# eblerjana/pangenie

Hardware: AMD Instinct MI355X
Metric: genotyped variants/sec (whole node) at H haplotypes; HBM GB/s vs roofline (higher is better)
Workload: dtype f64

## Files before the change

### pangenie_amd/csrc/pg_experiments.h

```cpp
#pragma once

#ifndef PG_EXP
#define PG_EXP 0
#endif
static constexpr unsigned kExp = PG_EXP;
#ifdef PG_CHAIN_PROF
static constexpr bool kChainProf = true;
#else
static constexpr bool kChainProf = false;
#endif

#ifndef PG_LEAN_EXP
#define PG_LEAN_EXP 0
#endif
static constexpr unsigned kLeanExp = PG_LEAN_EXP;
#ifndef PG_LEAN_UPKEEP_EXP
#define PG_LEAN_UPKEEP_EXP 0
#endif
static constexpr unsigned kLeanUpkeepExp = PG_LEAN_UPKEEP_EXP;
#ifdef PG_LEAN_DPPSUM
static constexpr bool kLeanDppSum = true;
#else
static constexpr bool kLeanDppSum = false;
#endif

#ifdef PG_POST_GENERIC
static constexpr bool kPostGeneric = true;
#else
static constexpr bool kPostGeneric = false;
#endif

#ifndef PG_PERSIST_EXP
#define PG_PERSIST_EXP 0
#endif
static constexpr unsigned kPersistExp = PG_PERSIST_EXP;

#ifndef PG_LEAN_PRETOTAL
#define PG_LEAN_PRETOTAL 0
#endif
static constexpr bool kLeanPreTotal = PG_LEAN_PRETOTAL != 0;

#ifdef PG_NT_STORES
static constexpr bool kNtStores = true;
#else
static constexpr bool kNtStores = false;
#endif
#ifdef PG_NT_POST
static constexpr bool kNtPost = true;
#else
static constexpr bool kNtPost = false;
#endif

#ifndef PG_LX_EXP
#define PG_LX_EXP 0
#endif
static constexpr unsigned kLxExp = PG_LX_EXP;

#ifndef PG_LEANP_EXP
#define PG_LEANP_EXP 0
#endif
static constexpr unsigned kLeanpExp = PG_LEANP_EXP;

#ifdef PG_LEAN_TIMELINE
static constexpr bool kLeanTimeline = true;
#else
static constexpr bool kLeanTimeline = false;
#endif
struct LeanTimeline {
    unsigned long long t[10], acc[10];
    DEVI void init() { if constexpr (kLeanTimeline) { for (int i = 0; i < 10; ++i) { t[i] = 0; acc[i] = 0; } } }
    template <int I>
    DEVI void mark(double dep) {
        if constexpr (kLeanTimeline) {
            __builtin_amdgcn_sched_barrier(0);
            asm volatile("" :: "v"(dep));
            t[I] = __builtin_amdgcn_s_memtime();
            __builtin_amdgcn_sched_barrier(0);
        }
    }
    template <int N>
    DEVI void fold() {
        if constexpr (kLeanTimeline) {
#pragma unroll
            for (int i = 0; i < N; ++i) acc[i] += t[i + 1] - t[i];
            acc[9] += 1;
        }
    }
    DEVI void write(unsigned long long* o) const {
        if constexpr (kLeanTimeline) { for (int i = 0; i < 9; ++i) o[i] = acc[i]; o[15] = acc[9]; }
    }
};

#ifndef PG_X_EXP
#define PG_X_EXP 0
#endif
static constexpr unsigned kXExp = PG_X_EXP;

#ifdef PG_VIT_TIMELINE
static constexpr bool kVitTimeline = true;
#else
static constexpr bool kVitTimeline = false;
#endif
// ... 38 lines not shown
```

### pangenie_amd/csrc/pg_kernels.hip

```cpp
#include <hip/hip_runtime.h>
#include <math.h>
#include <stdint.h>
#include <stdlib.h>

#include <type_traits>

#include "pg_device.h"
#include "pg_devmath.h"
#include "pg_launch.h"

#define DEVI __device__ __forceinline__
typedef double v2f64 __attribute__((ext_vector_type(2)));
#include "pg_experiments.h"

template <int CTRL, int ROW_MASK, bool BOUND>
DEVI double dpp_f64(double v) {
    int lo = __double2loint(v), hi = __double2hiint(v);
    lo = __builtin_amdgcn_update_dpp(0, lo, CTRL, ROW_MASK, 0xF, BOUND);
    hi = __builtin_amdgcn_update_dpp(0, hi, CTRL, ROW_MASK, 0xF, BOUND);
    return __hiloint2double(hi, lo);
}

DEVI double readlane_f64(double v, int src_lane ) {
    int lo = __builtin_amdgcn_readlane(__double2loint(v), src_lane);
// ... 2431 lines not shown
    static constexpr int NW = 64 / R;
    double psum[2][NW][64];
    double ptot[2][NW] __attribute__((aligned(32)));
    double u[NW][64] __attribute__((aligned(16)));
    double scal[2][64];
    double img[2 * PG_LEAN_BLOCK][PG_LEAN_IMAGE / 8] __attribute__((aligned(PG_LEAN_IMAGE)));
};
static_assert(PG_LEAN_IMAGE == 256 && (2 * PG_LEAN_BLOCK * PG_LEAN_IMAGE & (2 * PG_LEAN_BLOCK * PG_LEAN_IMAGE - 1)) == 0, "image(rel): a shift and a mask");
constexpr uint32_t kLeanImgTab = 64u, kLeanImgComb = 192u;
template <class SH>
DEVI LAS const unsigned char* lean_image(const SH& sh, uint32_t rel ) {
    static_assert(sizeof(sh.img) == 2u * PG_LEAN_SPARSE * PG_LEAN_IMAGE, "pg_lean_ring_image");
    return (LAS const unsigned char*)&sh.img[0][0] + pg_lean_ring_image(rel);
}
struct FRec {
    double c0, c1, c2, kappa, E00, E01, E11;
    unsigned long long bits1;
};
typedef double v4f64 __attribute__((ext_vector_type(4)));
struct LeanRecs {
    const GAS char* base;
    int64_t origin, C;
    int dir;
    uint32_t tid;
    DEVI v2f64 fetch(uint32_t block) const {
        int64_t c = origin + (int64_t)dir * ((int64_t)block * PG_LEAN_BLOCK + ((tid & 255u) >> 2));
        c = c < 0 ? 0 : (c >= C ? C - 1 : c);
        return *(const GAS v2f64*)(base + (size_t)c * 64u + (tid & 3u) * 16u);
    }
    template <class SH>
    DEVI void park(SH& sh, uint32_t block, v2f64 piece) const {
        if (tid < 256u) *(v2f64*)&sh.img[(block & 1u) * PG_LEAN_BLOCK + (tid >> 2)][(tid & 3u) * 2u] = piece;
    }
};
template <class SH>
DEVI FRec read_frec(const SH& sh, uint32_t rel ) {
    LAS const double* q = (LAS const double*)lean_image(sh, rel);
    FRec r;
    r.c0 = q[0]; r.c1 = q[1]; r.c2 = q[2]; r.kappa = q[3]; r.E00 = q[4]; r.E01 = q[5]; r.E11 = q[6];
    r.bits1 = (unsigned long long)__double_as_longlong(q[7]);
    return r;
}

DEVI double wave_total_mfma(double v) {
    const v4f64 z = {0.0, 0.0, 0.0, 0.0};
    const v4f64 a = __builtin_amdgcn_mfma_f64_16x16x4f64(v, 1.0, z, 0, 0, 0);
    const double u = (a[0] + a[1]) + (a[2] + a[3]);
    const v4f64 b = __builtin_amdgcn_mfma_f64_16x16x4f64(u, 1.0, z, 0, 0, 0);
    return b[0];
}
DEVI double sel_by_bit(uint32_t bits , int k, double if0, double if1) {
    const uint32_t m = (uint32_t)(((int32_t)(bits << (31 - k))) >> 31);
    const uint32_t lo = ((uint32_t)__double2loint(if1) & m) | ((uint32_t)__double2loint(if0) & ~m);
    const uint32_t hi = ((uint32_t)__double2hiint(if1) & m) | ((uint32_t)__double2hiint(if0) & ~m);
    return __hiloint2double((int)hi, (int)lo);
}

struct ColScalars {
    double* row;
    unsigned long long valid = 0ull;
    DEVI void put(uint32_t , uint64_t t , double v ) {
        row[t & 63u] = v;
        valid |= 1ull << (t & 63u);
    }
    DEVI void flush(gdouble* arr, uint32_t lane, uint64_t t_any ) {
        if ((valid >> lane) & 1ull) arr[(t_any & ~(uint64_t)63u) + lane] = row[lane];
        valid = 0ull;
    }
};

template <int R>
DEVI void lean_u_rows(double urep, double (&ui)[R]) {
    static_assert(R == 16, "one DPP row of 16 lanes = the wave's 16 rows");
    ui[0] = row_bcast_f64<0>(urep);   ui[1] = row_bcast_f64<1>(urep);   ui[2] = row_bcast_f64<2>(urep);   ui[3] = row_bcast_f64<3>(urep);
    ui[4] = row_bcast_f64<4>(urep);   ui[5] = row_bcast_f64<5>(urep);   ui[6] = row_bcast_f64<6>(urep);   ui[7] = row_bcast_f64<7>(urep);
    ui[8] = row_bcast_f64<8>(urep);   ui[9] = row_bcast_f64<9>(urep);   ui[10] = row_bcast_f64<10>(urep); ui[11] = row_bcast_f64<11>(urep);
    ui[12] = row_bcast_f64<12>(urep); ui[13] = row_bcast_f64<13>(urep); ui[14] = row_bcast_f64<14>(urep); ui[15] = row_bcast_f64<15>(urep);
}
template <int K>
DEVI double fmac_row_bcast(double acc, double u, double s) {
    asm("v_fmac_f64_dpp %0, %1, %2 row_newbcast:%3 row_mask:0xf bank_mask:0xf" : "+v"(acc) : "v"(u), "v"(s), "n"(K));
    return acc;
}
DEVI void pin_here(double& v) { asm volatile("" : "+v"(v)); }
DEVI void lean_fence() { __builtin_amdgcn_sched_barrier(0); }
DEVI double dpp_source(double v) {
    double r;
    asm("v_mov_b64 %0, %1\n\ts_nop 1" : "=v"(r) : "v"(v));
    return r;
}
template <int K>
DEVI unsigned long long row_mask64(unsigned long long bits ) {
    unsigned long long m;
    asm("s_bfe_i64 %0, %1, %2" : "=s"(m) : "s"(bits), "n"((1 << 16) | K) : "scc");
    return m;
}
DEVI double sel_by_mask(double if0, double if1, unsigned long long m ) {
    uint32_t lo, hi;
    asm("v_cndmask_b32_e64 %0, %1, %2, %3" : "=v"(lo) : "v"(__double2loint(if0)), "v"(__double2loint(if1)), "s"(m));
    asm("v_cndmask_b32_e64 %0, %1, %2, %3" : "=v"(hi) : "v"(__double2hiint(if0)), "v"(__double2hiint(if1)), "s"(m));
    return __hiloint2double((int)hi, (int)lo);
}
template <int K, int N, class F>
DEVI void static_for(F&& f) {
    if constexpr (K < N) { f(std::integral_constant<int, K>{}); static_for<K + 1, N>(f); }
}
template <int SEL>
DEVI uint32_t add_byte(uint32_t bytes, uint32_t base) {
    uint32_t r;
    if constexpr (SEL == 0) asm("v_add_u32_sdwa %0, %1, %2 dst_sel:DWORD dst_unused:UNUSED_PAD src0_sel:BYTE_0 src1_sel:DWORD" : "=v"(r) : "v"(bytes), "v"(base));
    else if constexpr (SEL == 1) asm("v_add_u32_sdwa %0, %1, %2 dst_sel:DWORD dst_unused:UNUSED_PAD src0_sel:BYTE_1 src1_sel:DWORD" : "=v"(r) : "v"(bytes), "v"(base));
    else if constexpr (SEL == 2) asm("v_add_u32_sdwa %0, %1, %2 dst_sel:DWORD dst_unused:UNUSED_PAD src0_sel:BYTE_2 src1_sel:DWORD" : "=v"(r) : "v"(bytes), "v"(base));
    else asm("v_add_u32_sdwa %0, %1, %2 dst_sel:DWORD dst_unused:UNUSED_PAD src0_sel:BYTE_3 src1_sel:DWORD" : "=v"(r) : "v"(bytes), "v"(base));
    return r;
}
template <class SH>
DEVI void lean_expand(SH& sh, uint32_t block , uint32_t tid) {
    static_assert(sizeof(sh.img[0]) == PG_LEAN_IMAGE && kLeanImgComb + 4u * 8u <= PG_LEAN_IMAGE, "four waves of eight row pairs");
    if (tid >= 256u) return;
    double* im = sh.img[(block & 1u) * PG_LEAN_BLOCK + (tid >> 2)];
    {
        const uint32_t c = tid & 3u;
        const double E00 = im[4], E01 = im[5], E11 = im[6];
        v2f64* tab = (v2f64*)((unsigned char*)im + kLeanImgTab);
        tab[c * 2u + 0u] = v2f64{(c & 1u) ? E01 : E00, (c & 2u) ? E01 : E00};
        tab[c * 2u + 1u] = v2f64{(c & 1u) ? E11 : E01, (c & 2u) ? E11 : E01};
    }
    {
        const uint32_t w = tid & 3u;
        const unsigned long long bits = (unsigned long long)__double_as_longlong(im[7]);
        const uint32_t b16 = (uint32_t)(bits >> (16u * w)) & 0xFFFFu;
        auto spread = [](uint32_t v8) { return ((v8 & 3u) | (((v8 >> 2) & 3u) << 8) | (((v8 >> 4) & 3u) << 16) | (((v8 >> 6) & 3u) << 24)) << 5; };
        typedef uint32_t u32x2 __attribute__((ext_vector_type(2)));
        *(u32x2*)((unsigned char*)im + kLeanImgComb + w * 8u) = u32x2{spread(b16 & 0xFFu), spread(b16 >> 8)};
    }
}
struct LeanPairs { uint32_t tbase, cd0, cd1; };
typedef uint32_t u32x2 __attribute__((ext_vector_type(2)));
template <class SH>
DEVI u32x2 lean_pair_bytes(const SH& sh, uint32_t rel , uint32_t wave ) {
    return *(LAS const u32x2*)(lean_image(sh, rel) + kLeanImgComb + wave * 8u);
}
template <class SH>
DEVI LeanPairs lean_pairs(const SH& sh, uint32_t rel , u32x2 cd, uint32_t aj ) {
    return LeanPairs{(uint32_t)(uintptr_t)lean_image(sh, rel) + kLeanImgTab + aj * 16u, cd.x, cd.y};
}
template <class SH>
DEVI LeanPairs lean_pairs(const SH& sh, uint32_t rel, uint32_t wave, uint32_t aj) { return lean_pairs(sh, rel, lean_pair_bytes(sh, rel, wave), aj); }
template <int P>
DEVI v2f64 lean_pair(const LeanPairs& lp) {
    return *(LAS const v2f64*)(uintptr_t)add_byte<(P & 3)>(P < 4 ? lp.cd0 : lp.cd1, lp.tbase);
}
template <int R>
DEVI void lean_pairs_all(const LeanPairs& lp, double (&e)[R]) {
    static_for<0, R / 2>([&](auto pc) __attribute__((always_inline)) { constexpr int q = decltype(pc)::value; const v2f64 t = lean_pair<q>(lp); e[2 * q] = t.x; e[2 * q + 1] = t.y; });
}
template <class SH>
DEVI v2f64 lean_ring_open(SH& sh, const LeanRecs& recs, uint32_t s0 , uint32_t tid) {
    const bool two = s0 > PG_LEAN_RING_PARK;
    recs.park(sh, 0, recs.fetch(0));
    v2f64 piece = recs.fetch(1);
    if (two) {
        lds_barrier();
        lean_expand(sh, 0, tid);
        lds_barrier();
        recs.park(sh, 1, piece);
// ... 13 lines not shown
            recs.park(sh, blk, piece);
            piece = recs.fetch(blk + 1u);
        } else if (((n + 3u) % PG_LEAN_BLOCK) == 0u) {
            lean_expand(sh, (n + 3u) / PG_LEAN_BLOCK, tid);
        }
    } else if constexpr (UPKEEP == kUpkeepPark) {
        const uint32_t blk = (n + 4u) / PG_LEAN_BLOCK;
        recs.park(sh, blk, piece);
        piece = recs.fetch(blk + 1u);
    } else if constexpr (UPKEEP == kUpkeepExpand) {
        lean_expand(sh, (n + 3u) / PG_LEAN_BLOCK, tid);
    }
}
template <int R>
DEVI double lean_colsum(const LeanShared<R>& sh, uint32_t pb, uint32_t lane) {
    if constexpr (R == 16)
        return (sh.psum[pb][0][lane] + sh.psum[pb][1][lane]) + (sh.psum[pb][2][lane] + sh.psum[pb][3][lane]);
    else
        return ((sh.psum[pb][0][lane] + sh.psum[pb][1][lane]) + (sh.psum[pb][2][lane] + sh.psum[pb][3][lane])) +
               ((sh.psum[pb][4][lane] + sh.psum[pb][5][lane]) + (sh.psum[pb][6][lane] + sh.psum[pb][7][lane]));
}



#define PG_SYNC_TIMEOUT_TICKS 1000000000ull
#ifndef PG_POLL_SLEEPS
#define PG_POLL_SLEEPS 2
#endif
DEVI bool chunk_spin(uint32_t* flag, uint32_t want, uint32_t* err) {
    bool ok = __hip_atomic_load(flag, __ATOMIC_RELAXED, __HIP_MEMORY_SCOPE_AGENT) >= want;
    if (!ok) {
        const unsigned long long t0 = wall_clock64();
        for (uint32_t it = 0;; ++it) {
#pragma unroll
            for (int z = 0; z < PG_POLL_SLEEPS; ++z) __builtin_amdgcn_s_sleep(127);
            if (__hip_atomic_load(flag, __ATOMIC_RELAXED, __HIP_MEMORY_SCOPE_AGENT) >= want) { ok = true; break; }
            if ((it & 63u) == 63u) {
                if (__hip_atomic_load(err, __ATOMIC_RELAXED, __HIP_MEMORY_SCOPE_AGENT) & PG_DEVERR_SYNC_TIMEOUT) break;
                if (wall_clock64() - t0 > PG_SYNC_TIMEOUT_TICKS) { atomicOr(err, PG_DEVERR_SYNC_TIMEOUT); break; }
            }
        }
    }
    if (ok) __builtin_amdgcn_fence(__ATOMIC_ACQUIRE, "agent");
    return ok;
}
DEVI void chunk_publish(uint32_t* flag, uint32_t value) {
    __builtin_amdgcn_fence(__ATOMIC_RELEASE, "agent");
    __syncthreads();
    if (threadIdx.x == 0) __hip_atomic_store(flag, value, __ATOMIC_RELEASE, __HIP_MEMORY_SCOPE_AGENT);
}
DEVI void chunk_wait_buffer(uint32_t* flag, uint32_t want, uint32_t* err) {
    if (threadIdx.x == 0 && !(kPersistExp & 2u)) (void)chunk_spin(flag, want, err);
    __syncthreads();
}

DEVI void lean_store(gdouble2* p, v2f64 v) {
    if constexpr (kNtStores) __builtin_nontemporal_store(v, p);
    else *p = v;
}
template <int R>
DEVI void lean_put_sums(LeanShared<R>& sh, uint32_t pb, uint32_t wave, uint32_t lane, double part) {
    sh.psum[pb][wave][lane] = part;
    if constexpr (kLeanPreTotal) {
        double v = part;
        v += dpp_f64<0x111, 0xF, true>(v);
        v += dpp_f64<0x112, 0xF, true>(v);
        v += dpp_f64<0x114, 0xF, true>(v);
        v += dpp_f64<0x118, 0xF, true>(v);
        v += dpp_f64<0x142, 0xA, false>(v);
        v += dpp_f64<0x143, 0xC, false>(v);
        if (lane == 63u) sh.ptot[pb][wave] = v;
    }
}
template <int R>
DEVI double lean_total(const LeanShared<R>& sh, uint32_t pb) {
    static_assert(R == 16, "four waves");
    const v2f64 a = *(const v2f64*)&sh.ptot[pb][0], b = *(const v2f64*)&sh.ptot[pb][2];
    return (a.x + a.y) + (b.x + b.y);
}

template <int PHASE, int R, bool TRI, bool SPARSE = false>
DEVI void lean_forward(const DevContig& dc, LeanShared<R>& sh, uint32_t C, uint32_t chunk) {
    static_assert(!SPARSE || ((PHASE == 1 || PHASE == 3) && !TRI), "sparse stores: phases 1 and 3 of full-column lean chains");
    constexpr int HP = 64;
    constexpr uint32_t RMASK = (1u << R) - 1u;
    const uint32_t mid = C / 2, K = dc.chunk_cols;
    uint32_t lo = PHASE == 1 ? 0u : mid, hi = PHASE == 1 ? mid : C;
    if constexpr (PHASE == 3) {
        const unsigned long long l = (unsigned long long)mid + (unsigned long long)chunk * K;
        if (l >= C) return;
        lo = (uint32_t)l;
        hi = C - lo > K ? lo + K : C;
    }
    if constexpr (SPARSE && PHASE == 1) if (chunk) {
        uint32_t pc[2];
        if (!pg_sparse_piece(C, 0u, (chunk >> 16) * K, chunk & 0xFFFFu, pc)) return;
        lo = pc[0]; hi = pc[1] + 1u;
    }
    bool seg2 = false;
    if constexpr (PHASE == 5) {
        lo = chunk + 1u; hi = chunk + PG_LEAN_SPARSE;
        seg2 = lo >= mid;
        if (seg2) hi = C - lo > PG_LEAN_SPARSE ? lo + PG_LEAN_SPARSE : C;
    }
    if (lo >= hi) return;
    const uint32_t first = lo == 0 ? 1u : lo;
    const uint32_t tid = threadIdx.x, lane = tid & 63u;
    const uint32_t wave = __builtin_amdgcn_readfirstlane(tid >> 6);
    const uint32_t i0 = wave * R;
    const size_t colsz = TRI ? (size_t)dc.col_stride : (size_t)HP * HP;
    const double unif = 1.0 / 4096.0;
    const uint32_t s0 = SPARSE ? pg_lean_ring_first(pg_lean_ring_lead(C, 0u, (uint32_t)PHASE, first, hi)) : 0u;
    LeanRecs recs{(const GAS char*)dc.frec, (int64_t)first - 1 - (int64_t)s0, (int64_t)C, +1, tid};
    v2f64 piece = lean_ring_open(sh, recs, s0, tid);
    gdouble* fwd = (gdouble*)dc.fwd;
    gdouble* fscale = (gdouble*)dc.fscale;
    gu8* fallback = (gu8*)dc.fwd_fallback;
    gdouble* wr = fwd;
    gcdouble* resume = (gcdouble*)(fwd + (size_t)(lo > 0 ? lo - 1 : 0) * colsz);
    if constexpr (PHASE == 3) {
        gdouble* scr = (gdouble*)dc.scratch;
        wr = scr + (size_t)(PG_SCR_BUF(chunk) * 2u) * K * colsz - (size_t)lo * colsz;
        if constexpr (SPARSE) { if (chunk > 0) resume = (gcdouble*)dc.ckpt + (size_t)(lo - mid) / PG_LEAN_SPARSE * colsz; }
        else if (chunk > 0) resume = (gcdouble*)(scr + ((size_t)(PG_SCR_BUF(chunk - 1u) * 2u) * K + (K - 1u)) * colsz);
    }
    if constexpr (PHASE == 4) wr = (gdouble*)dc.scratch - (size_t)lo * colsz;
    bool boundary = false;
    if constexpr (PHASE == 5) if (seg2) {
        const uint32_t m = (lo - mid) / PG_LEAN_SPARSE, ci = (lo - mid) / K;
        if (m) resume = (gcdouble*)dc.ckpt + (size_t)m * colsz;
        wr = (gdouble*)dc.scratch + (size_t)(PG_SCR_BUF(ci) * 2u) * K * colsz - ((size_t)mid + (size_t)ci * K) * colsz;
        boundary = (lo - mid) % K == 0u;
    }
    const size_t toff = (size_t)(i0 >> 1) * HP + lane;
    auto emis = [&](const FRec& r, double& eA, double& eB) {
        const bool aj = (r.bits1 >> lane) & 1ull;
        eA = aj ? r.E01 : r.E00;
        eB = aj ? r.E11 : r.E01;
    };
    double tfa[TRI ? R / 2 : 1], tfb[TRI ? R / 2 : 1];
    uint32_t tskip = 0, tunit[TRI ? R / 2 : 1];
    uint32_t rskip = 0;
    if constexpr (PHASE == 5) {
#pragma unroll
        for (int q = 0; q < R / 2; ++q) rskip |= (lane < ((i0 + 2u * (uint32_t)q) & ~7u) ? 1u : 0u) << q;
    }
    if constexpr (TRI) {
#pragma unroll
        for (int q = 0; q < R / 2; ++q) {
            const uint32_t r0 = i0 + 2u * (uint32_t)q;
            tfa[q] = lane < r0 ? 0.0 : (lane == r0 ? 0.5 : 1.0);
            tfb[q] = lane <= r0 ? 0.0 : (lane == r0 + 1u ? 0.5 : 1.0);
            const bool off_q = lane < (r0 & ~7u);
            tskip |= (off_q ? 1u : 0u) << q;
            tunit[q] = off_q ? 0u : tri_unit_of(r0 >> 1, lane);
        }
    }
    auto put_pair = [&](gdouble2* dst, int q, double a, double b) __attribute__((always_inline)) {
        if constexpr (TRI) {
            if (!((tskip >> q) & 1u)) lean_store((dst - toff) + tunit[q], v2f64{a * tfa[q], b * tfb[q]});
        } else if constexpr (PHASE == 5) {
            if (!((rskip >> q) & 1u)) lean_store(dst + (size_t)q * HP, v2f64{a, b});
        } else {
            lean_store(dst + (size_t)q * HP, v2f64{a, b});
        }
    };
    auto col_at = [&](uint32_t c) __attribute__((always_inline)) -> gdouble* {
        if constexpr (SPARSE && PHASE == 3) return (gdouble*)dc.ckpt + (size_t)((c - (mid - 1u)) / PG_LEAN_SPARSE) * colsz;
        else return wr + (size_t)c * colsz;
    };
    auto store_col = [&](uint32_t c, const double (&v)[R]) {
        gdouble2* dst = (gdouble2*)col_at(c) + toff;
#pragma unroll
        for (int k = 0; k < R; k += 2) put_pair(dst, k >> 1, v[k], v[k + 1]);
    };
    auto flag_uniform = [&](uint32_t cprev) {
        bool stored = cprev >= lo;
        if constexpr (SPARSE && PHASE == 1) stored = pg_sparse_stored(C, 0u, cprev);
        if constexpr (SPARSE && PHASE == 3) stored = stored && pg_sparse2_stored(C, 0u, cprev);
        if (stored) {
            double xu[R];
#pragma unroll
            for (int k = 0; k < R; ++k) xu[k] = unif;
            store_col(cprev, xu);
        }
        if constexpr (PHASE != 5) if (wave == 0) fallback[cprev] = 1;
    };

    uint32_t noscal = ~0u;
    if constexpr (PHASE == 5) if (seg2 && pg_sparse2_stored(C, 0u, hi - 1u)) noscal = hi - 1u;
    ColScalars fsc{&sh.scal[0][0]};
    double x[R];
    {
        const FRec r0 = read_frec(sh, s0);
        double eA, eB;
        emis(r0, eA, eB);
        const uint32_t rb = (uint32_t)__builtin_amdgcn_readfirstlane((int)((uint32_t)(r0.bits1 >> i0) & RMASK));
        double part = 0.0;
        if (lo == 0) {
            const double P0 = ldexp(1.0, PG_BIAS_F);
            double pz[R];
#pragma unroll
            for (int k = 0; k < R; ++k) { pz[k] = P0; x[k] = sel_by_bit(rb, k, eA, eB) * P0; part += x[k]; }
            store_col(0, pz);
            if (wave == 0) fscale[0] = 1.0;
        } else {
            gcdouble2* src = (gcdouble2*)resume + toff;
#pragma unroll
            for (int k = 0; k < R; k += 2) { const v2f64 t = src[(size_t)(k >> 1) * HP]; x[k] = t.x; x[k + 1] = t.y; }
            if (!fallback[lo - 1]) {
#pragma unroll
                for (int k = 0; k < R; ++k) { const double e = sel_by_bit(rb, k, eA, eB); part = fma(e, x[k], part); x[k] *= e; }
            } else if ((PHASE == 5 && !boundary) || (SPARSE && PHASE == 1)) {
#pragma unroll
                for (int k = 0; k < R; ++k) x[k] = 0.0;
            } else {
#pragma unroll
                for (int k = 0; k < R; ++k) part += x[k];
            }
        }
        lean_put_sums<R>(sh, (first - 1) & 1u, wave, lane, part);
    }
    double ec[R];
    {
        const FRec r1 = read_frec(sh, s0 + 1u);
        lean_pairs_all<R>(lean_pairs(sh, s0 + 1u, wave, (uint32_t)((r1.bits1 >> lane) & 1ull)), ec);
    }
    LeanTimeline tl;
    tl.init();
    auto step = [&](auto store_c, auto upkeep_c, uint32_t t, const FRec& cur, FRec& nxt) __attribute__((always_inline)) {
        constexpr bool STORE = decltype(store_c)::value;
        constexpr int UPKEEP = decltype(upkeep_c)::value;
        const uint32_t n = t - first + s0;
        tl.template mark<0>(0.0);
        u32x2 cdn;
        auto next_record = [&]() __attribute__((always_inline)) {
            nxt = read_frec(sh, n + 2u);
            cdn = lean_pair_bytes(sh, n + 2u, wave);
            lean_ring_upkeep<UPKEEP>(sh, recs, piece, n, tid);
        };
        if constexpr (kLeanUpkeepExp & 2u) next_record();
        const uint32_t pb = (t - 1) & 1u;
        double pc[64 / R], pr[64 / R];
#pragma unroll
        for (int q = 0; q < 64 / R; ++q) { pc[q] = sh.psum[pb][q][lane]; pr[q] = sh.psum[pb][q][i0 + (lane & 15u)]; }
        const double Spre = kLeanPreTotal ? lean_total<R>(sh, pb) : 0.0;
        if constexpr (!(kLeanUpkeepExp & 2u)) {
            lean_fence();
            next_record();
            lean_fence();
        }
        const double Cj = (pc[0] + pc[1]) + (pc[2] + pc[3]);
        tl.template mark<1>(Cj);
        const v4f64 zz = {0.0, 0.0, 0.0, 0.0};
        const v4f64 ma = (kLeanDppSum || kLeanPreTotal) ? zz : __builtin_amdgcn_mfma_f64_16x16x4f64(Cj, 1.0, zz, 0, 0, 0);
        lean_fence();
        const double ucol = cur.c1 * Cj;
        const double urep = dpp_source(cur.c1 * ((pr[0] + pr[1]) + (pr[2] + pr[3])));
        const LeanPairs lp = lean_pairs(sh, n + 2u, cdn, (uint32_t)((nxt.bits1 >> lane) & 1ull));
        const double msum = (ma[0] + ma[1]) + (ma[2] + ma[3]);
        tl.template mark<2>(msum);
        lean_fence();
        const v4f64 mb = (kLeanDppSum || kLeanPreTotal) ? zz : __builtin_amdgcn_mfma_f64_16x16x4f64(msum, 1.0, zz, 0, 0, 0);
        if constexpr (!kLeanPreTotal) asm volatile("" :: "v"(mb));
        lean_fence();
        double S = (kLeanExp & 4) ? 64.0 * Cj : (kLeanPreTotal ? Spre : (kLeanDppSum ? wave_sum(Cj) : mb[0]));
        tl.template mark<3>(S);
        double uj = fma(cur.c2, S, ucol);
        double c0 = cur.c0;
        if (__builtin_expect(!(S > 0.0), 0)) {
            flag_uniform(t - 1);
            const double Cu = 64.0 * unif;
            S = 1.0;
            uj = fma(cur.c0, unif, fma(cur.c2, 1.0, 2.0 * cur.c1 * Cu));
            c0 = 0.0;
        }
        int es = exponent_of(S) - PG_BIAS_F;
        es = es < -900 ? -900 : es;
        const double m = ldexp(S, -es - PG_BIAS_F);
        const double sc = ldexp(1.0, -es), c0s = ldexp(c0, -es), ujs = ldexp(uj, -es);
        tl.template mark<4>(c0s + ujs + sc);
        gdouble2* dst = (gdouble2*)col_at(t) + toff;
        double part = 0.0, pprev = 0.0;
        static_for<0, R>([&](auto kc) __attribute__((always_inline)) {
            constexpr int k = decltype(kc)::value;
            const double pk = fmac_row_bcast<k>(fma(c0s, x[k], ujs), urep, sc);
            part = fma(ec[k], pk, part);
            x[k] = ec[k] * pk;
            pin_here(x[k]);
            if constexpr (k == 1) tl.template mark<5>(x[1]);
            if constexpr (k & 1) {
                if constexpr (STORE) { if (!(kLeanExp & 1)) put_pair(dst, k >> 1, pprev, pk); }
                const v2f64 t2 = (kLeanExp & 2) ? v2f64{0.5, 0.5} : lean_pair<(k >> 1)>(lp);
                ec[k - 1] = t2.x; ec[k] = t2.y;
                __builtin_amdgcn_sched_barrier(0);
            } else pprev = pk;
        });
        tl.template mark<6>(part);
        lean_put_sums<R>(sh, t & 1u, wave, lane, part);
        if constexpr (SPARSE) {
            if constexpr (STORE) if (wave == 0) fscale[t] = m;
        } else if (wave == 0) {
            if (PHASE != 5 || t != noscal) fsc.put(lane, t, m);
            if ((t & 63u) == 63u) fsc.flush(fscale, lane, t);
        }
        tl.template mark<7>(0.0);
        lds_barrier();
        tl.template mark<8>(0.0);
        tl.template fold<8>();
    };
    FRec ra = read_frec(sh, s0 + 1u), rb2;
    constexpr std::true_type kStore{};
    constexpr std::false_type kNoStore{};
    constexpr std::integral_constant<int, kUpkeepTested> kTested{};
    constexpr std::integral_constant<int, kUpkeepNone> kNone{};
    constexpr std::integral_constant<int, kUpkeepPark> kPark{};
    constexpr std::integral_constant<int, kUpkeepExpand> kExpand{};
    __builtin_amdgcn_s_waitcnt(0x0F70);
    lds_barrier();
    uint32_t t = first;
    if constexpr (PHASE == 4) {
        const uint32_t post_groups = 2u * (uint32_t)K;
        gdouble* scr = (gdouble*)dc.scratch;
        uint32_t q = 0, cend = hi - lo > K ? lo + K : hi;
        for (;;) {
            for (; t + 1 < cend; t += 2) {
                step(kStore, kTested, t, ra, rb2);
                step(kStore, kTested, t + 1, rb2, ra);
            }
            if (t < cend) { step(kStore, kTested, t, ra, rb2); ++t; }
            if (wave == 0 && fsc.valid) fsc.flush(fscale, lane, cend - 1);
            {
                const double Cj = lean_colsum<R>(sh, (cend - 1) & 1u, lane);
                if (!(wave_total_mfma(Cj) > 0.0)) flag_uniform(cend - 1);
            }
            chunk_publish(dc.sync + 0, q + 1u);
            if (cend >= hi) break;
            ++q;
            lo = cend;
            cend = hi - lo > K ? lo + K : hi;
            wr = scr + (size_t)(PG_SCR_BUF(q) * 2u) * K * colsz - (size_t)lo * colsz;
            if (q >= PG_SCRATCH_BUFS) chunk_wait_buffer(dc.sync + PG_SYNC_DONE + PG_SCR_BUF(q), (q / PG_SCRATCH_BUFS) * post_groups, dc.err);
        }
        return;
    }
    if constexpr (SPARSE) {
        if constexpr (PHASE == 1) {
            const uint32_t ck0 = (hi - 1u) % PG_LEAN_SPARSE;
            for (; t + 1 <= ck0; t += 2) {
                step(kStore, kTested, t, ra, rb2);
                step(kStore, kTested, t + 1, rb2, ra);
            }
            if (t <= ck0) { step(kStore, kTested, t, ra, rb2); ra = rb2; ++t; }
        }
        static_assert(PG_LEAN_SPARSE == PG_LEAN_BLOCK && PG_LEAN_RING_PARK % 2u == 0u && PG_LEAN_RING_EXPAND == PG_LEAN_RING_PARK + 1u && PG_LEAN_RING_PARK + 4u == PG_LEAN_SPARSE, "the group's last four steps: park, expand, plain, store");
        while (hi - t >= PG_LEAN_SPARSE) {
            for (uint32_t g = 0; g < PG_LEAN_RING_PARK / 2u; ++g, t += 2) {
                step(kNoStore, kNone, t, ra, rb2);
                step(kNoStore, kNone, t + 1, rb2, ra);
            }
            step(kNoStore, kPark, t, ra, rb2);
            step(kNoStore, kExpand, t + 1, rb2, ra);
            step(kNoStore, kNone, t + 2, ra, rb2);
            step(kStore, kNone, t + 3, rb2, ra);
            t += 4;
        }
        if constexpr (PHASE == 3) {
            for (; t + 1 < hi; t += 2) {
                step(kNoStore, kTested, t, ra, rb2);
                step(kNoStore, kTested, t + 1, rb2, ra);
            }
            if (t < hi) step(kNoStore, kTested, t, ra, rb2);
        }
    } else {
        for (; t + 1 < hi; t += 2) {
            step(kStore, kTested, t, ra, rb2);
            step(kStore, kTested, t + 1, rb2, ra);
        }
        if (t < hi) step(kStore, kTested, t, ra, rb2);
    }
    if constexpr (!SPARSE) if (wave == 0 && fsc.valid) fsc.flush(fscale, lane, hi - 1);
    if (kLeanTimeline && tid == 0) tl.write(dc.prof + 32);
    {
        const uint32_t pb = (hi - 1) & 1u;
        const double Cj = lean_colsum<R>(sh, pb, lane);
        if (!(wave_total_mfma(Cj) > 0.0)) flag_uniform(hi - 1);
    }
}

template <int PHASE, int R, bool TRI, bool SPARSE = false>
DEVI void lean_backward(const DevContig& dc, LeanShared<R>& sh, uint32_t C, uint32_t chunk) {
    static_assert(!SPARSE || ((PHASE == 1 || PHASE == 3) && !TRI), "sparse stores: phases 1 and 3 of full-column lean chains");
    constexpr int HP = 64;
    constexpr uint32_t RMASK = (1u << R) - 1u;
    const int64_t mid = C / 2, K = dc.chunk_cols;
    int64_t top = PHASE == 1 ? (int64_t)C - 1 : mid - 1;
    int64_t bot = PHASE == 1 ? mid : 0;
    if constexpr (PHASE == 3) {
        top = mid - 1 - (int64_t)chunk * K;
        if (top < 0) return;
        bot = top - K + 1 > 0 ? top - K + 1 : 0;
    }
    bool seg2 = false;
    if constexpr (PHASE == 5) {
        top = (int64_t)chunk - 1; bot = (int64_t)chunk - (int64_t)(PG_LEAN_SPARSE - 1u);
        seg2 = (int64_t)chunk <= mid;
        if (seg2) bot = top + 1 > (int64_t)PG_LEAN_SPARSE ? top + 1 - (int64_t)PG_LEAN_SPARSE : 0;
    }
    bool resumed = PHASE != 1;
    if constexpr (SPARSE && PHASE == 1) if (chunk) {
        uint32_t pc[2];
        if (!pg_sparse_piece(C, 1u, (chunk >> 16) * dc.chunk_cols, chunk & 0xFFFFu, pc)) return;
        bot = pc[0]; top = pc[1];
        resumed = top != (int64_t)C - 1;
    }
    if (top < bot) return;
    const int64_t t0 = resumed ? top : top - 1;
    const uint32_t tid = threadIdx.x, lane = tid & 63u;
    const uint32_t wave = __builtin_amdgcn_readfirstlane(tid >> 6);
    const uint32_t i0 = wave * R;
    const size_t colsz = TRI ? (size_t)dc.col_stride : (size_t)HP * HP;
    const double unif = 1.0 / 4096.0;
    const uint32_t s0 = SPARSE && t0 >= bot ? pg_lean_ring_first(pg_lean_ring_lead(C, 1u, (uint32_t)PHASE, (uint32_t)t0, (uint32_t)bot)) : 0u;
    LeanRecs recs{(const GAS char*)dc.frec, t0 + 1 + (int64_t)s0, (int64_t)C, -1, tid};
    v2f64 piece = lean_ring_open(sh, recs, s0, tid);
    gdouble* cols = (gdouble*)dc.fwd;
    gdouble* bscale = (gdouble*)dc.bscale;
    gdouble* bsum = (gdouble*)dc.bsum;
    gdouble* wr = cols;
    gcdouble* resume = (gcdouble*)(cols + (size_t)(top + 1 < (int64_t)C ? top + 1 : top) * colsz);
    if constexpr (PHASE == 3) {
        gdouble* scr = (gdouble*)dc.scratch;
        wr = scr + (size_t)(PG_SCR_BUF(chunk) * 2u + 1u) * (size_t)K * colsz - (size_t)bot * colsz;
        if constexpr (SPARSE) { if (chunk > 0) resume = (gcdouble*)dc.ckpt + ((size_t)dc.ckpt_slots + (size_t)(mid - 1 - top) / PG_LEAN_SPARSE) * colsz; }
        else if (chunk > 0) resume = (gcdouble*)(scr + (size_t)(PG_SCR_BUF(chunk - 1u) * 2u + 1u) * (size_t)K * colsz);
    }
    if constexpr (PHASE == 5) if (seg2) {
        const size_t m = (size_t)(mid - 1 - top) / PG_LEAN_SPARSE;
        const int64_t ci = (mid - 1 - top) / K, ctop = mid - 1 - ci * K;
        if (m) resume = (gcdouble*)dc.ckpt + ((size_t)dc.ckpt_slots + m) * colsz;
        wr = (gdouble*)dc.scratch + (size_t)(PG_SCR_BUF((uint32_t)ci) * 2u + 1u) * (size_t)K * colsz - (size_t)(ctop - K + 1 > 0 ? ctop - K + 1 : 0) * colsz;
    }
    int64_t cbot = bot;
    if constexpr (PHASE == 4) {
        cbot = top - K + 1 > 0 ? top - K + 1 : 0;
        wr = (gdouble*)dc.scratch + (size_t)K * colsz - (size_t)cbot * colsz;
    }
    const size_t toff = (size_t)(i0 >> 1) * HP + lane;
    auto emis = [&](const FRec& r, double& eA, double& eB) {
        const bool aj = (r.bits1 >> lane) & 1ull;
        eA = aj ? r.E01 : r.E00;
        eB = aj ? r.E11 : r.E01;
    };
    double tfa[TRI ? R / 2 : 1], tfb[TRI ? R / 2 : 1];
    uint32_t tskip = 0, tunit[TRI ? R / 2 : 1];
    uint32_t rskip = 0;
    if constexpr (PHASE == 5) {
#pragma unroll
        for (int q = 0; q < R / 2; ++q) rskip |= (lane < ((i0 + 2u * (uint32_t)q) & ~7u) ? 1u : 0u) << q;
    }
    if constexpr (TRI) {
#pragma unroll
        for (int q = 0; q < R / 2; ++q) {
            const uint32_t r0 = i0 + 2u * (uint32_t)q;
            tfa[q] = lane < r0 ? 0.0 : (lane == r0 ? 0.5 : 1.0);
            tfb[q] = lane <= r0 ? 0.0 : (lane == r0 + 1u ? 0.5 : 1.0);
            const bool off_q = lane < (r0 & ~7u);
            tskip |= (off_q ? 1u : 0u) << q;
            tunit[q] = off_q ? 0u : tri_unit_of(r0 >> 1, lane);
        }
    }
    auto put_pair = [&](gdouble2* dst, int q, double a, double b) __attribute__((always_inline)) {
        if constexpr (TRI) {
            if (!((tskip >> q) & 1u)) lean_store((dst - toff) + tunit[q], v2f64{a * tfa[q], b * tfb[q]});
// ... 2 lines not shown
        } else {
            lean_store(dst + (size_t)q * HP, v2f64{a, b});
        }
    };
    auto col_at = [&](int64_t c) __attribute__((always_inline)) -> gdouble* {
        if constexpr (SPARSE && PHASE == 3) return (gdouble*)dc.ckpt + ((size_t)dc.ckpt_slots + (size_t)(mid - c) / PG_LEAN_SPARSE) * colsz;
        else return wr + (size_t)c * colsz;
    };
    auto store_col = [&](int64_t c, const double (&v)[R]) {
        gdouble2* dst = (gdouble2*)col_at(c) + toff;
#pragma unroll
        for (int k = 0; k < R; k += 2) put_pair(dst, k >> 1, v[k], v[k + 1]);
    };

    int64_t noscal = -1;
    if constexpr (PHASE == 5) if (seg2 && pg_sparse2_stored(C, 1u, (uint32_t)bot)) noscal = bot;
    ColScalars bsc{&sh.scal[0][0]}, bsm{&sh.scal[1][0]};
    double w[R], Sy;
    FRec cur = read_frec(sh, s0);
    {
        double y[R];
        if (!resumed) {
            const double B0 = ldexp(1.0, PG_BIAS_B);
#pragma unroll
            for (int k = 0; k < R; ++k) y[k] = B0;
            Sy = 4096.0 * B0;
            store_col(top, y);
            if (wave == 0) { bscale[top] = 1.0; bsum[top] = Sy; }
        } else {
            gcdouble2* src = (gcdouble2*)resume + toff;
#pragma unroll
            for (int k = 0; k < R; k += 2) { const v2f64 t = src[(size_t)(k >> 1) * HP]; y[k] = t.x; y[k + 1] = t.y; }
            Sy = bsum[top + 1];
            if (!(Sy > 0.0)) {
#pragma unroll
                for (int k = 0; k < R; ++k) y[k] = unif;
                Sy = 1.0;
            }
        }
        double eA, eB;
        emis(cur, eA, eB);
        const uint32_t rb = (uint32_t)__builtin_amdgcn_readfirstlane((int)((uint32_t)(cur.bits1 >> i0) & RMASK));
        double part = 0.0;
#pragma unroll
        for (int k = 0; k < R; ++k) { const double e = sel_by_bit(rb, k, eA, eB); part = fma(e, y[k], part); w[k] = y[k] * e; }
        lean_put_sums<R>(sh, (uint32_t)t0 & 1u, wave, lane, part);
    }
    double ec[R];
    {
        const FRec r1 = read_frec(sh, s0 + 1u);
        lean_pairs_all<R>(lean_pairs(sh, s0 + 1u, wave, (uint32_t)((r1.bits1 >> lane) & 1ull)), ec);
    }
    double one = 1.0;
    asm volatile("" : "+v"(one));
    LeanTimeline tl;
    tl.init();
    auto step = [&](auto store_c, auto upkeep_c, int64_t t, const FRec& cur, FRec& nxt) __attribute__((always_inline)) {
        constexpr bool STORE = decltype(store_c)::value;
        constexpr int UPKEEP = decltype(upkeep_c)::value;
        const uint32_t n = (uint32_t)(t0 - t) + s0;
        tl.template mark<0>(0.0);
        lean_ring_upkeep<UPKEEP>(sh, recs, piece, n, tid);
        int es = exponent_of(Sy) - PG_BIAS_B;
        es = es < -900 ? -900 : es;
        const double m = ldexp(Sy, -es - PG_BIAS_B);
        if constexpr (SPARSE) {
            if constexpr (STORE) if (wave == 1) { asm volatile("" ::: "memory"); bscale[t] = m; }
        } else if (wave == 1 && (PHASE != 5 || t != noscal)) { asm volatile("" ::: "memory"); bsc.put(lane, (uint64_t)t, m); }
        double k0 = ldexp(cur.c0, -es), k1 = ldexp(cur.c1, -es), k2 = ldexp(cur.c2, -es), kap = ldexp(cur.kappa, -es);
        pin_here(k0); pin_here(k1); pin_here(k2); pin_here(kap);
        tl.template mark<1>(k0 + kap);
        lds_barrier();
        tl.template mark<2>(0.0);
        const uint32_t pb = (uint32_t)t & 1u;
        double pc[64 / R], pr[64 / R];
#pragma unroll
        for (int q = 0; q < 64 / R; ++q) { pc[q] = sh.psum[pb][q][lane]; pr[q] = sh.psum[pb][q][i0 + (lane & 15u)]; }
        const double Spre = kLeanPreTotal ? lean_total<R>(sh, pb) : 0.0;
        lean_fence();
        nxt = read_frec(sh, n + 1u);
        const unsigned long long bits_n = (unsigned long long)__double_as_longlong(((LAS const double*)lean_image(sh, n + 2u))[7]);
        const u32x2 cdn = lean_pair_bytes(sh, n + 2u, wave);
        lean_fence();
        const double Cj = (pc[0] + pc[1]) + (pc[2] + pc[3]);
        tl.template mark<3>(Cj);
        const v4f64 zz = {0.0, 0.0, 0.0, 0.0};
        const v4f64 ma = (kLeanDppSum || kLeanPreTotal) ? zz : __builtin_amdgcn_mfma_f64_16x16x4f64(Cj, 1.0, zz, 0, 0, 0);
        lean_fence();
        const double ucol = k1 * Cj;
        const double urep = dpp_source(k1 * ((pr[0] + pr[1]) + (pr[2] + pr[3])));
        const LeanPairs lp = lean_pairs(sh, n + 2u, cdn, (uint32_t)((bits_n >> lane) & 1ull));
        const double msum = (ma[0] + ma[1]) + (ma[2] + ma[3]);
        tl.template mark<4>(msum);
        lean_fence();
        const v4f64 mb = (kLeanDppSum || kLeanPreTotal) ? zz : __builtin_amdgcn_mfma_f64_16x16x4f64(msum, 1.0, zz, 0, 0, 0);
        if constexpr (!kLeanPreTotal) asm volatile("" :: "v"(mb));
        lean_fence();
        const double Sw = (kLeanExp & 4) ? 64.0 * Cj : (kLeanPreTotal ? Spre : (kLeanDppSum ? wave_sum(Cj) : mb[0]));
        tl.template mark<5>(Sw);
        const double uj = fma(k2, Sw, ucol);
        const double Snew = kap * Sw;
        Sy = Snew;
        gdouble2* dst = (gdouble2*)col_at(t) + toff;
        double part = 0.0, yprev = 0.0;
        const bool zero = !(Snew > 0.0);
        static_for<0, R>([&](auto kc) __attribute__((always_inline)) {
            constexpr int k = decltype(kc)::value;
            const double yk = fmac_row_bcast<k>(fma(k0, w[k], uj), urep, one);
            part = fma(ec[k], yk, part);
            w[k] = ec[k] * yk;
            pin_here(w[k]);
            if constexpr (k == 1) tl.template mark<6>(w[1]);
            if constexpr (k & 1) {
                if constexpr (STORE) { if (!(kLeanExp & 1)) put_pair(dst, k >> 1, yprev, yk); }
                const v2f64 t2 = (kLeanExp & 2) ? v2f64{0.5, 0.5} : lean_pair<(k >> 1)>(lp);
                ec[k - 1] = t2.x; ec[k] = t2.y;
                __builtin_amdgcn_sched_barrier(0);
            } else yprev = yk;
        });
        if (__builtin_expect(zero, 0)) {
            double et[R];
            lean_pairs_all<R>(lean_pairs(sh, n + 1u, wave, (uint32_t)((nxt.bits1 >> lane) & 1ull)), et);
            part = 0.0;
#pragma unroll
            for (int k = 0; k < R; ++k) { w[k] = unif * et[k]; part += w[k]; }
            Sy = 1.0;
        }
        tl.template mark<7>(part);
        lean_put_sums<R>(sh, (uint32_t)(t - 1) & 1u, wave, lane, part);
        if constexpr (SPARSE) {
            if constexpr (STORE) if (wave == 2) { asm volatile("" ::: "memory"); bsum[t] = Snew; }
        } else if constexpr (PHASE != 5) {
            if (wave == 2) { asm volatile("" ::: "memory"); bsm.put(lane, (uint64_t)t, Snew); }
            if (((uint64_t)t & 63u) == 0u) {
                if (wave == 1) bsc.flush(bscale, lane, (uint64_t)t);
                if (wave == 2) bsm.flush(bsum, lane, (uint64_t)t);
            }
        } else {
            if (wave == 1 && ((uint64_t)t & 63u) == 0u) bsc.flush(bscale, lane, (uint64_t)t);
        }
        tl.template mark<8>(0.0);
        tl.template fold<8>();
    };
    FRec rb2;
    constexpr std::true_type kStore{};
    constexpr std::false_type kNoStore{};
    constexpr std::integral_constant<int, kUpkeepTested> kTested{};
    constexpr std::integral_constant<int, kUpkeepNone> kNone{};
    constexpr std::integral_constant<int, kUpkeepPark> kPark{};
    constexpr std::integral_constant<int, kUpkeepExpand> kExpand{};
    int64_t t = t0;
    __builtin_amdgcn_s_waitcnt(0x0F70);
    if constexpr (PHASE == 4) {
        const uint32_t post_groups = 2u * (uint32_t)K;
        gdouble* scr = (gdouble*)dc.scratch;
        uint32_t q = 0;
        for (;;) {
            for (; t - 1 >= cbot; t -= 2) {
                step(kStore, kTested, t, cur, rb2);
                step(kStore, kTested, t - 1, rb2, cur);
            }
            if (t >= cbot) { step(kStore, kTested, t, cur, rb2); --t; }
            if (wave == 1 && bsc.valid) bsc.flush(bscale, lane, (uint64_t)cbot);
            if (wave == 2 && bsm.valid) bsm.flush(bsum, lane, (uint64_t)cbot);
            chunk_publish(dc.sync + 1, q + 1u);
            if (cbot == 0) break;
            ++q;
            const int64_t ntop = cbot - 1;
            cbot = ntop - K + 1 > 0 ? ntop - K + 1 : 0;
            wr = scr + (size_t)(PG_SCR_BUF(q) * 2u + 1u) * (size_t)K * colsz - (size_t)cbot * colsz;
            if (q >= PG_SCRATCH_BUFS) chunk_wait_buffer(dc.sync + PG_SYNC_DONE + PG_SCR_BUF(q), (q / PG_SCRATCH_BUFS) * post_groups, dc.err);
        }
        return;
    }
    if constexpr (SPARSE) {
        if constexpr (PHASE == 1) {
            const int64_t ckh = mid + (int64_t)pg_sparse_segments(C, 1u) * (int64_t)PG_LEAN_SPARSE;
            for (; t - 1 >= ckh; t -= 2) {
                step(kStore, kTested, t, cur, rb2);
                step(kStore, kTested, t - 1, rb2, cur);
            }
            if (t >= ckh) { step(kStore, kTested, t, cur, rb2); cur = rb2; --t; }
        }
        while (t - bot >= (int64_t)PG_LEAN_SPARSE - 1) {
            for (uint32_t g = 0; g < PG_LEAN_RING_PARK / 2u; ++g, t -= 2) {
                step(kNoStore, kNone, t, cur, rb2);
                step(kNoStore, kNone, t - 1, rb2, cur);
            }
            step(kNoStore, kPark, t, cur, rb2);
            step(kNoStore, kExpand, t - 1, rb2, cur);
            step(kNoStore, kNone, t - 2, cur, rb2);
// ... 3109 lines not shown
```

Before: 27.12 million.

## Hoist row-broadcast update into MFMA reduction latency window in lean chains

The per-row broadcast term (c0*x + urow broadcast) is now computed before the column total is available, filling the latency of the two serial MFMA reductions. The default mode (split 2) does all 16 rows as plain fma with a row broadcast before the second MFMA. Mode 1 fuses the DPP fmacs into an inline-asm block right behind the MFMA. The post-total loop then only adds the scalar uj term, which shortens the dependent critical path per column. This adds hand-scheduled asm and register pressure. The scaling by sc is also reordered, which could change rounding slightly.

```diff
diff --git a/pangenie_amd/csrc/pg_experiments.h b/pangenie_amd/csrc/pg_experiments.h
--- a/pangenie_amd/csrc/pg_experiments.h
+++ b/pangenie_amd/csrc/pg_experiments.h
@@ -18,6 +18,14 @@
 #define PG_LEAN_UPKEEP_EXP 0
 #endif
 static constexpr unsigned kLeanUpkeepExp = PG_LEAN_UPKEEP_EXP;
+#ifndef PG_LEAN_SPLIT
+#define PG_LEAN_SPLIT 2
+#endif
+static constexpr int kLeanSplit = PG_LEAN_SPLIT;
+#ifndef PG_LEAN_SPLIT_HEAD
+#define PG_LEAN_SPLIT_HEAD 16
+#endif
+static constexpr int kLeanSplitHead = PG_LEAN_SPLIT_HEAD;
 #ifdef PG_LEAN_DPPSUM
 static constexpr bool kLeanDppSum = true;
 #else
diff --git a/pangenie_amd/csrc/pg_kernels.hip b/pangenie_amd/csrc/pg_kernels.hip
--- a/pangenie_amd/csrc/pg_kernels.hip
+++ b/pangenie_amd/csrc/pg_kernels.hip
@@ -2537,6 +2537,23 @@
     asm("v_fmac_f64_dpp %0, %1, %2 row_newbcast:%3 row_mask:0xf bank_mask:0xf" : "+v"(acc) : "v"(u), "v"(s), "n"(K));
     return acc;
 }
+DEVI v4f64 mfma_total_rows(double a, double u, double s, double (&x)[16]) {
+    v4f64 d;
+    asm volatile("s_nop 1\n\tv_mfma_f64_16x16x4_f64 %0, %17, %19, 0\n\t"
+                 "v_fmac_f64_dpp %1, %18, %19 row_newbcast:0 row_mask:0xf bank_mask:0xf\n\tv_fmac_f64_dpp %2, %18, %19 row_newbcast:1 row_mask:0xf bank_mask:0xf\n\t"
+                 "v_fmac_f64_dpp %3, %18, %19 row_newbcast:2 row_mask:0xf bank_mask:0xf\n\tv_fmac_f64_dpp %4, %18, %19 row_newbcast:3 row_mask:0xf bank_mask:0xf\n\t"
+                 "v_fmac_f64_dpp %5, %18, %19 row_newbcast:4 row_mask:0xf bank_mask:0xf\n\tv_fmac_f64_dpp %6, %18, %19 row_newbcast:5 row_mask:0xf bank_mask:0xf\n\t"
+                 "v_fmac_f64_dpp %7, %18, %19 row_newbcast:6 row_mask:0xf bank_mask:0xf\n\tv_fmac_f64_dpp %8, %18, %19 row_newbcast:7 row_mask:0xf bank_mask:0xf\n\t"
+                 "v_fmac_f64_dpp %9, %18, %19 row_newbcast:8 row_mask:0xf bank_mask:0xf\n\tv_fmac_f64_dpp %10, %18, %19 row_newbcast:9 row_mask:0xf bank_mask:0xf\n\t"
+                 "v_fmac_f64_dpp %11, %18, %19 row_newbcast:10 row_mask:0xf bank_mask:0xf\n\tv_fmac_f64_dpp %12, %18, %19 row_newbcast:11 row_mask:0xf bank_mask:0xf\n\t"
+                 "v_fmac_f64_dpp %13, %18, %19 row_newbcast:12 row_mask:0xf bank_mask:0xf\n\tv_fmac_f64_dpp %14, %18, %19 row_newbcast:13 row_mask:0xf bank_mask:0xf\n\t"
+                 "v_fmac_f64_dpp %15, %18, %19 row_newbcast:14 row_mask:0xf bank_mask:0xf\n\tv_fmac_f64_dpp %16, %18, %19 row_newbcast:15 row_mask:0xf bank_mask:0xf\n\t"
+                 "s_nop 2"
+                 : "=&v"(d), "+v"(x[0]), "+v"(x[1]), "+v"(x[2]), "+v"(x[3]), "+v"(x[4]), "+v"(x[5]), "+v"(x[6]), "+v"(x[7]), "+v"(x[8]), "+v"(x[9]), "+v"(x[10]),
+                   "+v"(x[11]), "+v"(x[12]), "+v"(x[13]), "+v"(x[14]), "+v"(x[15])
+                 : "v"(a), "v"(u), "v"(s));
+    return d;
+}
 DEVI void pin_here(double& v) { asm volatile("" : "+v"(v)); }
 DEVI void lean_fence() { __builtin_amdgcn_sched_barrier(0); }
 DEVI double dpp_source(double v) {
@@ -2716,6 +2733,7 @@
 template <int PHASE, int R, bool TRI, bool SPARSE = false>
 DEVI void lean_forward(const DevContig& dc, LeanShared<R>& sh, uint32_t C, uint32_t chunk) {
     static_assert(!SPARSE || ((PHASE == 1 || PHASE == 3) && !TRI), "sparse stores: phases 1 and 3 of full-column lean chains");
+    constexpr int SPLIT = TRI ? 0 : kLeanSplit, HEAD = kLeanSplitHead;
     constexpr int HP = 64;
     constexpr uint32_t RMASK = (1u << R) - 1u;
     const uint32_t mid = C / 2, K = dc.chunk_cols;
@@ -2860,6 +2878,8 @@
         const FRec r1 = read_frec(sh, s0 + 1u);
         lean_pairs_all<R>(lean_pairs(sh, s0 + 1u, wave, (uint32_t)((r1.bits1 >> lane) & 1ull)), ec);
     }
+    double one = 1.0;
+    if constexpr (SPLIT == 1) asm volatile("" : "+v"(one));
     LeanTimeline tl;
     tl.init();
     auto step = [&](auto store_c, auto upkeep_c, uint32_t t, const FRec& cur, FRec& nxt) __attribute__((always_inline)) {
@@ -2884,18 +2904,37 @@
             next_record();
             lean_fence();
         }
+        if constexpr (SPLIT == 1) {
+#pragma unroll
+            for (int k = 0; k < R; ++k) { x[k] = cur.c0 * x[k]; pin_here(x[k]); }
+            lean_fence();
+        }
         const double Cj = (pc[0] + pc[1]) + (pc[2] + pc[3]);
         tl.template mark<1>(Cj);
         const v4f64 zz = {0.0, 0.0, 0.0, 0.0};
         const v4f64 ma = (kLeanDppSum || kLeanPreTotal) ? zz : __builtin_amdgcn_mfma_f64_16x16x4f64(Cj, 1.0, zz, 0, 0, 0);
         lean_fence();
         const double ucol = cur.c1 * Cj;
-        const double urep = dpp_source(cur.c1 * ((pr[0] + pr[1]) + (pr[2] + pr[3])));
+        const double urow = cur.c1 * ((pr[0] + pr[1]) + (pr[2] + pr[3]));
+        const double urep = SPLIT == 2 ? urow : dpp_source(urow);
         const LeanPairs lp = lean_pairs(sh, n + 2u, cdn, (uint32_t)((nxt.bits1 >> lane) & 1ull));
+        if constexpr (SPLIT == 2) static_for<0, HEAD>([&](auto kc) __attribute__((always_inline)) {
+            constexpr int k = decltype(kc)::value;
+            x[k] = fma(cur.c0, x[k], row_bcast_f64<k>(urep)); pin_here(x[k]);
+        });
         const double msum = (ma[0] + ma[1]) + (ma[2] + ma[3]);
         tl.template mark<2>(msum);
         lean_fence();
-        const v4f64 mb = (kLeanDppSum || kLeanPreTotal) ? zz : __builtin_amdgcn_mfma_f64_16x16x4f64(msum, 1.0, zz, 0, 0, 0);
+        v4f64 mb = zz;
+        if constexpr (SPLIT == 1 && !kLeanDppSum && !kLeanPreTotal) mb = mfma_total_rows(msum, urep, one, x);
+        else {
+            if constexpr (!kLeanDppSum && !kLeanPreTotal) mb = __builtin_amdgcn_mfma_f64_16x16x4f64(msum, 1.0, zz, 0, 0, 0);
+            if constexpr (SPLIT == 1) static_for<0, R>([&](auto kc) __attribute__((always_inline)) { constexpr int k = decltype(kc)::value; x[k] = fmac_row_bcast<k>(x[k], urep, one); });
+            if constexpr (SPLIT == 2) static_for<HEAD, R>([&](auto kc) __attribute__((always_inline)) {
+                constexpr int k = decltype(kc)::value;
+                x[k] = fma(cur.c0, x[k], row_bcast_f64<k>(urep)); pin_here(x[k]);
+            });
+        }
         if constexpr (!kLeanPreTotal) asm volatile("" :: "v"(mb));
         lean_fence();
         double S = (kLeanExp & 4) ? 64.0 * Cj : (kLeanPreTotal ? Spre : (kLeanDppSum ? wave_sum(Cj) : mb[0]));
@@ -2912,13 +2951,13 @@
         int es = exponent_of(S) - PG_BIAS_F;
         es = es < -900 ? -900 : es;
         const double m = ldexp(S, -es - PG_BIAS_F);
-        const double sc = ldexp(1.0, -es), c0s = ldexp(c0, -es), ujs = ldexp(uj, -es);
+        const double sc = ldexp(1.0, -es), c0s = SPLIT ? 0.0 : ldexp(c0, -es), ujs = ldexp(uj, -es);
         tl.template mark<4>(c0s + ujs + sc);
         gdouble2* dst = (gdouble2*)col_at(t) + toff;
         double part = 0.0, pprev = 0.0;
         static_for<0, R>([&](auto kc) __attribute__((always_inline)) {
             constexpr int k = decltype(kc)::value;
-            const double pk = fmac_row_bcast<k>(fma(c0s, x[k], ujs), urep, sc);
+            const double pk = SPLIT ? fma(x[k], sc, ujs) : fmac_row_bcast<k>(fma(c0s, x[k], ujs), urep, sc);
             part = fma(ec[k], pk, part);
             x[k] = ec[k] * pk;
             pin_here(x[k]);
@@ -3024,6 +3063,7 @@
 
 template <int PHASE, int R, bool TRI, bool SPARSE = false>
 DEVI void lean_backward(const DevContig& dc, LeanShared<R>& sh, uint32_t C, uint32_t chunk) {
+    constexpr int SPLIT = TRI ? 0 : kLeanSplit, HEAD = kLeanSplitHead;
     static_assert(!SPARSE || ((PHASE == 1 || PHASE == 3) && !TRI), "sparse stores: phases 1 and 3 of full-column lean chains");
     constexpr int HP = 64;
     constexpr uint32_t RMASK = (1u << R) - 1u;
@@ -3192,18 +3232,37 @@
         const unsigned long long bits_n = (unsigned long long)__double_as_longlong(((LAS const double*)lean_image(sh, n + 2u))[7]);
         const u32x2 cdn = lean_pair_bytes(sh, n + 2u, wave);
         lean_fence();
+        if constexpr (SPLIT == 1) {
+#pragma unroll
+            for (int k = 0; k < R; ++k) { w[k] = k0 * w[k]; pin_here(w[k]); }
+            lean_fence();
+        }
         const double Cj = (pc[0] + pc[1]) + (pc[2] + pc[3]);
         tl.template mark<3>(Cj);
         const v4f64 zz = {0.0, 0.0, 0.0, 0.0};
         const v4f64 ma = (kLeanDppSum || kLeanPreTotal) ? zz : __builtin_amdgcn_mfma_f64_16x16x4f64(Cj, 1.0, zz, 0, 0, 0);
         lean_fence();
         const double ucol = k1 * Cj;
-        const double urep = dpp_source(k1 * ((pr[0] + pr[1]) + (pr[2] + pr[3])));
+        const double urow = k1 * ((pr[0] + pr[1]) + (pr[2] + pr[3]));
+        const double urep = SPLIT == 2 ? urow : dpp_source(urow);
         const LeanPairs lp = lean_pairs(sh, n + 2u, cdn, (uint32_t)((bits_n >> lane) & 1ull));
+        if constexpr (SPLIT == 2) static_for<0, HEAD>([&](auto kc) __attribute__((always_inline)) {
+            constexpr int k = decltype(kc)::value;
+            w[k] = fma(k0, w[k], row_bcast_f64<k>(urep)); pin_here(w[k]);
+        });
         const double msum = (ma[0] + ma[1]) + (ma[2] + ma[3]);
         tl.template mark<4>(msum);
         lean_fence();
-        const v4f64 mb = (kLeanDppSum || kLeanPreTotal) ? zz : __builtin_amdgcn_mfma_f64_16x16x4f64(msum, 1.0, zz, 0, 0, 0);
+        v4f64 mb = zz;
+        if constexpr (SPLIT == 1 && !kLeanDppSum && !kLeanPreTotal) mb = mfma_total_rows(msum, urep, one, w);
+        else {
+            if constexpr (!kLeanDppSum && !kLeanPreTotal) mb = __builtin_amdgcn_mfma_f64_16x16x4f64(msum, 1.0, zz, 0, 0, 0);
+            if constexpr (SPLIT == 1) static_for<0, R>([&](auto kc) __attribute__((always_inline)) { constexpr int k = decltype(kc)::value; w[k] = fmac_row_bcast<k>(w[k], urep, one); });
+            if constexpr (SPLIT == 2) static_for<HEAD, R>([&](auto kc) __attribute__((always_inline)) {
+                constexpr int k = decltype(kc)::value;
+                w[k] = fma(k0, w[k], row_bcast_f64<k>(urep)); pin_here(w[k]);
+            });
+        }
         if constexpr (!kLeanPreTotal) asm volatile("" :: "v"(mb));
         lean_fence();
         const double Sw = (kLeanExp & 4) ? 64.0 * Cj : (kLeanPreTotal ? Spre : (kLeanDppSum ? wave_sum(Cj) : mb[0]));
@@ -3216,7 +3275,7 @@
         const bool zero = !(Snew > 0.0);
         static_for<0, R>([&](auto kc) __attribute__((always_inline)) {
             constexpr int k = decltype(kc)::value;
-            const double yk = fmac_row_bcast<k>(fma(k0, w[k], uj), urep, one);
+            const double yk = SPLIT ? w[k] + uj : fmac_row_bcast<k>(fma(k0, w[k], uj), urep, one);
             part = fma(ec[k], yk, part);
             w[k] = ec[k] * yk;
             pin_here(w[k]);
```

After: 27.41 million, median of 6. +1.1%, better.
